# kyle-he/gym-comm

Hardware: AMD Instinct MI355X
Metric: env-steps/sec (whole node) (higher is better)
Workload: dtype int32

## Files before the change

gym-comm_amd/csrc/oc_step_device.h:

```cpp
#pragma once
#include <hip/hip_runtime.h>

#include <type_traits>

#include "../../include/oc_hip.h"
#include "oc_level_host.h"
#include "oc_policy_device.h"

namespace {

#ifdef OC_STAMPS
#define OC_STAMP(k)                                                                  \
  do {                                                                               \
    unsigned long long t_;                                                           \
    __builtin_amdgcn_sched_barrier(0);                                               \
    asm volatile("s_memtime %0\n\ts_waitcnt lgkmcnt(0)" : "=s"(t_)::"memory");     \
    __builtin_amdgcn_sched_barrier(0);                                               \
    oc_tt[(k)] = t_;                                                                 \
  } while (0)
#define OC_STAMP_PARAM , unsigned long long (&oc_tt)[16]
#define OC_STAMP_PASS , oc_tt
#else
#define OC_STAMP(k) do { } while (0)
#define OC_STAMP_PARAM
// ... 136 lines not shown
__device__ __forceinline__ P p_gt(int a, int b) { return p_lt(b, a); }
__device__ __forceinline__ P p_ge(int a, int b) { return ~p_lt(a, b); }
__device__ __forceinline__ P p_le(int a, int b) { return ~p_lt(b, a); }
__device__ __forceinline__ P p_eq_any(int a, int b) { return hide(a == b ? -1 : 0); }
__device__ __forceinline__ P p_gtu_any(unsigned a, unsigned b) { return hide(a > b ? -1 : 0); }
__device__ __forceinline__ P p_geu_any(unsigned a, unsigned b) { return hide(a >= b ? -1 : 0); }
__device__ __forceinline__ P p_ltu_any(unsigned a, unsigned b) { return hide(a < b ? -1 : 0); }
__device__ __forceinline__ P p_bit(int w, unsigned k) { return hide(__builtin_amdgcn_sbfe(w, k, 1u)); }
__device__ __forceinline__ P p_of(bool uniform) { return uniform ? -1 : 0; }
__device__ __forceinline__ int sel(P m, int a, int b) { return (a & m) | (b & ~m); }

__device__ __forceinline__ int iabs(int v) { return v < 0 ? -v : v; }
__device__ __forceinline__ unsigned sad_u32(unsigned a, unsigned b, unsigned c) {
  unsigned r;
  asm("v_sad_u32 %0, %1, %2, %3" : "=v"(r) : "v"(a), "v"(b), "v"(c));
  return r;
}
__device__ __forceinline__ int manhattan(int p, int q) {
  return (int)sad_u32((unsigned)(p & 15), (unsigned)(q & 15), sad_u32((unsigned)(p >> 4), (unsigned)(q >> 4), 0u));
}
__device__ __forceinline__ int px(int p) { return p & 15; }
__device__ __forceinline__ int py(int p) { return p >> 4; }
__device__ __forceinline__ int dense(const Hdr &L, int p) {
  return __mul24(py(p), L.W() - 16) + p;
}
__device__ __forceinline__ int bit128(uint64_t w0, uint64_t w1, int c) {
  const uint64_t v = (c & 64) ? w1 : w0;
  return (int)((v >> (c & 63)) & 1);
}
__device__ __forceinline__ int item_type(const Hdr &L, int i) { return (L.item_types() >> (4 * i)) & 15; }
__device__ __forceinline__ int cell_type(const Hdr &L, int c) {
  if (!L.planes128())
    return (int)((L.cell_lo(0) >> c) & 1) | ((int)((L.cell_hi(0) >> c) & 1) << 1);
  return bit128(L.cell_lo(0), L.cell_lo(1), c) | (bit128(L.cell_hi(0), L.cell_hi(1), c) << 1);
}

#ifdef OC_SPECIALIZED
constexpr bool OC_BORDER_CLOSED = OC_SPEC_HDR.closed_border != 0;
#else
constexpr bool OC_BORDER_CLOSED = false;
#endif

__device__ __forceinline__ double timestep_of(int t, const RunCfg &R) {
  typedef int v2i __attribute__((ext_vector_type(2)));
  const double dt = (double)t;
  const double q0 = dt * R.inv_T;
  const double r = __builtin_fma(-(double)R.T, q0, dt);
  const v2i q = __builtin_bit_cast(v2i, __builtin_fma(r, R.inv_T, q0));
  const P unlimited = p_of(R.T == 0);
  const int hi0 = 0x7FF00000 | (p_z(t) & 0x00080000);
  v2i out;
  out.x = q.x & ~unlimited;
  out.y = sel(unlimited, hi0, q.y);
  return __builtin_bit_cast(double, out);
}


template <int AUX>
struct RowsT {
  __amdgpu_buffer_rsrc_t rsrc;
  int voff;
  int rowbytes;
  __device__ __forceinline__ RowsT(const void *base, int64_t n, int rows, int64_t i, int elem = 4) {
    rsrc = __builtin_amdgcn_make_buffer_rsrc(const_cast<void *>(base), 0, (int)(n * rows * elem), 0x00020000);
    voff = (int)i * elem;
    rowbytes = (int)n * elem;
  }
  __device__ __forceinline__ int ld(int row) const {
    return __builtin_amdgcn_raw_buffer_load_b32(rsrc, voff, row * rowbytes, 0);
  }
  __device__ __forceinline__ void st(int row, int v) const {
    __builtin_amdgcn_raw_buffer_store_b32(v, rsrc, voff, row * rowbytes, AUX);
  }
  __device__ __forceinline__ void st8(int row, int v) const {
    __builtin_amdgcn_raw_buffer_store_b8((char)v, rsrc, voff, row * rowbytes, AUX);
  }
  __device__ __forceinline__ void st_f64(int row, double v) const {
    typedef int v2i __attribute__((ext_vector_type(2)));
    __builtin_amdgcn_raw_buffer_store_b64(__builtin_bit_cast(v2i, v), rsrc, voff, row * rowbytes, AUX);
  }
  __device__ __forceinline__ int soff(int row) const { return row * rowbytes; }
  __device__ __forceinline__ void st_at(int so, int, int v) const {
    __builtin_amdgcn_raw_buffer_store_b32(v, rsrc, voff, so, AUX);
  }
  __device__ __forceinline__ void st8_at(int so, int, int v) const {
    __builtin_amdgcn_raw_buffer_store_b8((char)v, rsrc, voff, so, AUX);
  }
};
template <int AUX, int N>
struct RowsPreT : RowsT<AUX> {
  int so[N > 0 ? N : 1];
  int row0;
  __device__ __forceinline__ RowsPreT(const RowsT<AUX> &rows, int row0_) : RowsT<AUX>(rows), row0(row0_) {
    [[maybe_unused]] int o = row0_ * rows.rowbytes;
#pragma unroll
    for (int k = 0; k < N; k++) {
      so[k] = o;
      asm volatile("" : "+s"(so[k]));
      o = so[k] + rows.rowbytes;
    }
  }
  __device__ __forceinline__ int off(int row) const {
    const int k = row - row0;
    return (k >= 0 && k < N) ? so[k] : row * this->rowbytes;
  }
  __device__ __forceinline__ void st(int row, int v) const {
    __builtin_amdgcn_raw_buffer_store_b32(v, this->rsrc, this->voff, off(row), AUX);
  }
  __device__ __forceinline__ void st8(int row, int v) const {
    __builtin_amdgcn_raw_buffer_store_b8((char)v, this->rsrc, this->voff, off(row), AUX);
  }
  __device__ __forceinline__ void st_v(int row, int vo, int v) const {
    __builtin_amdgcn_raw_buffer_store_b32(v, this->rsrc, vo, off(row), AUX);
  }
  __device__ __forceinline__ void st8_v(int row, int vo, int v) const {
    __builtin_amdgcn_raw_buffer_store_b8((char)v, this->rsrc, vo, off(row), AUX);
  }
};
template <int AUX, int OT>
struct RowsLdsT : RowsT<AUX> {
  float *lds;
  int rowbase, lane;
  __device__ __forceinline__ RowsLdsT(const RowsT<AUX> &rows, float *lds_, int rowbase_, int lane_)
      : RowsT<AUX>(rows), lds(lds_), rowbase(rowbase_), lane(lane_) {}
  __device__ __forceinline__ void st(int row, int v) const {
    RowsT<AUX>::st(row, v);
    lds[(row - rowbase) * 64 + lane] = OT == 2 ? __builtin_bit_cast(float, v) : (float)v;
  }
  __device__ __forceinline__ void st8(int row, int v) const {
    RowsT<AUX>::st8(row, v);
    lds[(row - rowbase) * 64 + lane] = (float)v;
  }
  __device__ __forceinline__ void st_at(int so, int row, int v) const {
    RowsT<AUX>::st_at(so, row, v);
    lds[(row - rowbase) * 64 + lane] = OT == 2 ? __builtin_bit_cast(float, v) : (float)v;
  }
  __device__ __forceinline__ void st8_at(int so, int row, int v) const {
    RowsT<AUX>::st8_at(so, row, v);
    lds[(row - rowbase) * 64 + lane] = (float)v;
  }
};
using Rows = RowsT<0>;
#ifndef OC_AUX_WT
#define OC_AUX_WT 16
#endif
constexpr int AUX_WT = OC_AUX_WT;

template <int B>
struct ShapeIn {
  int ap[B];
  int completed;
  int del_has[MAX_DELS], del_p[MAX_DELS];
  int chop_p[3];
};

template <int M>
__device__ __forceinline__ int pyset_first(const Hdr &L, const uint32_t *__restrict__ probe,
                                           const int (&iw)[M], const bool (&cand)[M], int &has) {
  constexpr int BIG = 1 << 20;
  int ord[M];
#pragma unroll
  for (int i = 0; i < M; i++)
    ord[i] = cand[i] ? (((iw[i] & IW_HOLD) ? 0 : 256) | ((iw[i] >> 16) & 255)) : BIG;
  int cell[3], code[3];
  bool valid[3];
  int prev = -1;
#pragma unroll
  for (int k = 0; k < 3; k++) {
    int cur = BIG, c = 0;
#pragma unroll
    for (int i = 0; i < M; i++) {
      const bool better = ord[i] > prev && ord[i] < cur;
      cur = better ? ord[i] : cur;
      c = better ? ipos(iw[i]) : c;
    }
    valid[k] = cur != BIG;
    cell[k] = c;
    prev = valid[k] ? cur : BIG;
  }
  has = valid[0];
  if (__ballot(valid[1]) == 0) return cell[0];
  valid[1] = valid[1] && cell[1] != cell[0];
  valid[2] = valid[2] && cell[2] != cell[0] && !(valid[1] && cell[2] == cell[1]);
#pragma unroll
  for (int k = 0; k < 3; k++) code[k] = valid[k] ? (int)probe[dense(L, cell[k])] : 0;
  const int s0 = code[0] & 7;
  int s1 = 8, s2 = 8;
#pragma unroll
  for (int t = 7; t >= 0; t--) {
    const int q1 = (code[1] >> (3 * t)) & 7;
    s1 = (q1 != s0) ? q1 : s1;
  }
  s1 = valid[1] ? s1 : 8;
#pragma unroll
  for (int t = 7; t >= 0; t--) {
    const int q2 = (code[2] >> (3 * t)) & 7;
    s2 = (q2 != s0 && q2 != s1) ? q2 : s2;
  }
  s2 = valid[2] ? s2 : 8;
  int best = cell[0], bs = s0;
  best = s1 < bs ? cell[1] : best;
  bs = min(bs, s1);
  best = s2 < bs ? cell[2] : best;
  return best;
}
template <int B>
struct ShapeLoads {
  int d_chop[3][B];
  int d_pair[MAX_PAIRLK];
  int d_del[MAX_DELS][B];
  int d_tile[OC_MAX_DELIV][B];
};

template <int B, int M, bool DUP>
__device__ __forceinline__ void shaping_issue_pos(const Hdr &L, const uint8_t *__restrict__ dist,
                                                  const ShapeIn<B> &in, const int (&ipos)[M], ShapeLoads<B> &ld) {
  const unsigned nc = (unsigned)L.ncells();
  unsigned arow[B];
#pragma unroll
  for (int b = 0; b < B; b++) arow[b] = __umul24((unsigned)dense(L, in.ap[b]), nc);
  unsigned ic[M];
#pragma unroll
  for (int i = 0; i < M; i++) ic[i] = (unsigned)dense(L, ipos[i]);
#pragma unroll
  for (int f = 0; f < 3; f++) {
#pragma unroll
    for (int b = 0; b < B; b++) ld.d_chop[f][b] = 0;
    if (L.chop_mask(f) != 0) {
      unsigned fc = 0;
      if constexpr (DUP) {
        fc = (unsigned)dense(L, in.chop_p[f]);
      } else {
#pragma unroll
        for (int i = 0; i < M; i++) fc = ((int)L.food_item(f) == i) ? ic[i] : fc;
      }
#pragma unroll
      for (int b = 0; b < B; b++) ld.d_chop[f][b] = dist[arow[b] + fc];
    }
  }
#pragma unroll
  for (int k = 0; k < MAX_PAIRLK; k++) {
    ld.d_pair[k] = 0;
    if (k < (int)L.npairlk()) {
      const int li = L.pairlk(k) & 15, lj = (L.pairlk(k) >> 4) & 15;
      unsigned ci = 0, cj = 0;
#pragma unroll
      for (int i = 0; i < M; i++) {
        ci = (li == i) ? ic[i] : ci;
        cj = (lj == i) ? ic[i] : cj;
      }
      ld.d_pair[k] = dist[__umul24(ci, nc) + cj];
    }
  }
#pragma unroll
  for (int k = 0; k < OC_MAX_DELIV; k++) {
#pragma unroll
    for (int b = 0; b < B; b++) ld.d_tile[k][b] = 0;
    if (k < (int)L.ndeliv()) {
      const unsigned dc = (unsigned)dense(L, (int)L.deliv_pos(k));
#pragma unroll
      for (int b = 0; b < B; b++) ld.d_tile[k][b] = dist[arow[b] + dc];
    }
  }
}

template <int B>
__device__ __forceinline__ void shaping_issue_del(const Hdr &L, const uint8_t *__restrict__ dist,
                                                  const ShapeIn<B> &in, ShapeLoads<B> &ld) {
  const unsigned nc = (unsigned)L.ncells();
#pragma unroll
  for (int k = 0; k < MAX_DELS; k++) {
#pragma unroll
    for (int b = 0; b < B; b++) ld.d_del[k][b] = 0;
    if (k < (int)L.ndel()) {
      const unsigned mc = (unsigned)dense(L, in.del_p[k]);
#pragma unroll
      for (int b = 0; b < B; b++) ld.d_del[k][b] = dist[__umul24((unsigned)dense(L, in.ap[b]), nc) + mc];
    }
  }
}

template <int B>
struct ShapeQ {
  double q_chop[B], q_pair, q_del[MAX_DELS][B];
  int nchop, npairs;
  bool del_direct[MAX_DELS][B];
};

__device__ __forceinline__ double quotient(int k, const Hdr &L, double inv_max_path) {
  const double dk = (double)k;
  const double q0 = dk * inv_max_path;
  const double r = __builtin_fma(-(double)L.max_path(), q0, dk);
  return __builtin_fma(r, inv_max_path, q0);
}

template <int B>
__device__ __forceinline__ void shaping_lookup(const Hdr &L, double inv_max_path, const ShapeIn<B> &in,
                                               const ShapeLoads<B> &ld, ShapeQ<B> &q OC_STAMP_PARAM) {
  const int MAXP = L.max_path();
  const int completed = in.completed;
  int d_tile[B];
#pragma unroll
  for (int b = 0; b < B; b++) d_tile[b] = 1 << 20;
#pragma unroll
  for (int k = 0; k < OC_MAX_DELIV; k++)
    if (k < (int)L.ndeliv()) {
#pragma unroll
      for (int b = 0; b < B; b++)
        d_tile[b] = min(d_tile[b], ld.d_tile[k][b] + manhattan(in.ap[b], (int)L.deliv_pos(k)));
    }
  int nchop = 0;
  int mind[B];
#pragma unroll
  for (int b = 0; b < B; b++) mind[b] = 1 << 20;
#pragma unroll
  for (int f = 0; f < 3; f++)
    if (L.chop_mask(f) != 0) {
      const int open = __popc((int)L.chop_mask(f) & ~completed);
      nchop += open;
#pragma unroll
      for (int b = 0; b < B; b++) mind[b] = open ? min(mind[b], ld.d_chop[f][b]) : mind[b];
    }
  int npairs = (int)L.pair_static_max();
  int minpair = npairs ? MAXP : (1 << 20);
  {
    int cur = MAXP;
#pragma unroll
    for (int k = 0; k < MAX_PAIRLK; k++)
      if (k < (int)L.npairlk()) {
        cur = min(cur, ld.d_pair[k]);
        if ((L.pairlk(k) >> 8) & 1) {
          const bool keep = cur != 0;
          npairs += keep ? 1 : 0;
          minpair = keep ? min(minpair, cur) : minpair;
          cur = MAXP;
        }
      }
  }
  int kq_chop[B], kq_pair;
#pragma unroll
  for (int b = 0; b < B; b++) kq_chop[b] = nchop ? (mind[b] + MAXP) + (nchop - 1) * 2 * MAXP : 0;
  kq_pair = nchop ? npairs * MAXP : (npairs ? minpair + (npairs - 1) * MAXP : 0);
  int kq_del[MAX_DELS][B];
#pragma unroll
  for (int k = 0; k < MAX_DELS; k++)
#pragma unroll
    for (int b = 0; b < B; b++) {
      kq_del[k][b] = 0;
      q.del_direct[k][b] = false;
      if (k < (int)L.ndel()) {
        const int d = ld.d_del[k][b] + manhattan(in.ap[b], in.del_p[k]);
        q.del_direct[k][b] = d == 0;
        kq_del[k][b] = d == 0 ? d_tile[b] : d;
      }
    }
#pragma unroll
  for (int b = 0; b < B; b++) q.q_chop[b] = quotient(kq_chop[b], L, inv_max_path);
  q.q_pair = quotient(kq_pair, L, inv_max_path);
#pragma unroll
  for (int k = 0; k < MAX_DELS; k++)
#pragma unroll
    for (int b = 0; b < B; b++) q.q_del[k][b] = (k < (int)L.ndel()) ? quotient(kq_del[k][b], L, inv_max_path) : 0.0;
  q.nchop = nchop;
  q.npairs = npairs;
  OC_STAMP(4);
}

template <int B>
__device__ __forceinline__ void shaping_sum(const Hdr &L, const ShapeIn<B> &in, const ShapeQ<B> &q,
                                            double &s0, double &s1 OC_STAMP_PARAM) {
  double tot[B];
#pragma unroll
  for (int b = 0; b < B; b++) {
    tot[b] = q.nchop ? q.q_chop[b] : 0.0;
    tot[b] = q.npairs ? tot[b] + q.q_pair : tot[b];
  }
#pragma unroll
  for (int k = 0; k < MAX_DELS; k++)
    if (k < (int)L.ndel()) {
      const bool open = !((in.completed >> L.del_bit(k)) & 1);
#pragma unroll
      for (int b = 0; b < B; b++) {
        const double add = !in.del_has[k] ? 2.0 : (q.del_direct[k][b] ? q.q_del[k][b] : q.q_del[k][b] + 1.0);
        tot[b] = open ? tot[b] + add : tot[b];
      }
    }
  s0 = tot[0];
  s1 = B > 1 ? tot[1] : 0.0;
  OC_STAMP(6);
}

template <int A, int M, bool DUP, int PM, bool FLAT>
__device__ __forceinline__ void env_step(const Hdr &L, const RunCfg &R, const uint8_t *__restrict__ dist,
                                         const uint32_t *__restrict__ probe,
                                         Env<A, M, DUP> &e, const int (&act_in)[A], int &reward, int &done, P &done_p,
                                         int &success, ShapeIn<(A < 2 ? A : 2)> &sin,
                                         ShapeLoads<(A < 2 ? A : 2)> &sld OC_STAMP_PARAM) {
  const int W = L.W(), H = L.H();
  const auto pb = [](int w, unsigned k) -> P {
    if constexpr (PM == 2 && FLAT) return __builtin_amdgcn_sbfe(w, k, 1u);
    return p_bit(w, k);
  };
  e.t = min(e.t + 1, 0xFFFF);
  static_assert(OC_ACT_NOOP == 4 && OC_FLOOR == 0 && OC_COUNTER == 1 && OC_CUTBOARD == 2 && OC_DELIVERY == 3, "codes");

  int act[A], np[A], tgt_p[A];
  P moving[A], t_nonfloor[A], t_deliv[A], t_cutb[A];
#pragma unroll
  for (int a = 0; a < A; a++) {
    int c = act_in[a];
    e.err |= p_gtu_any((unsigned)c, 4u) & OC_ERR_ACTION;
    c = (int)min((unsigned)c, 4u);
    act[a] = c;
    moving[a] = p_ne(c, OC_ACT_NOOP);
    int cell;
    P oob = 0;
    if constexpr (OC_BORDER_CLOSED) {
      constexpr uint64_t STEP = 0x0001FFF010ull;
      const int q = e.ap[a] + (int)(int8_t)(STEP >> (8 * c));
      tgt_p[a] = q;
      cell = dense(L, q);
    } else {
      const int dx = (c == OC_ACT_RIGHT) - (c == OC_ACT_LEFT);
      const int dy = (c == OC_ACT_DOWN) - (c == OC_ACT_UP);
      const int qx = px(e.ap[a]) + dx, qy = py(e.ap[a]) + dy;
      oob = ~(p_ltu_any((unsigned)qx, (unsigned)W) & p_ltu_any((unsigned)qy, (unsigned)H));
      e.err |= oob & OC_ERR_OOB;
      const int tx = min(max(qx, 0), W - 1), ty = min(max(qy, 0), H - 1);
      tgt_p[a] = tx | (ty << 4);
      cell = ty * W + tx;
    }
    P lo, hi;
    if (!L.planes128()) {
      lo = pb((int)(L.cell_lo(0) >> cell), 0);
      hi = pb((int)(L.cell_hi(0) >> cell), 0);
    } else {
      lo = -bit128(L.cell_lo(0), L.cell_lo(1), cell);
      hi = -bit128(L.cell_hi(0), L.cell_hi(1), cell);
    }
    t_nonfloor[a] = lo | hi;
    t_deliv[a] = lo & hi;
    t_cutb[a] = hi & ~lo;
    np[a] = sel(t_nonfloor[a] | oob, e.ap[a], tgt_p[a]);
  }
  P ex[A];
#pragma unroll
  for (int a = 0; a < A; a++) ex[a] = -1;
#pragma unroll
  for (int i = 0; i < A; i++)
#pragma unroll
    for (int j = i + 1; j < A; j++) {
      const P same = p_eq(np[i], np[j]);
      const P i_stays = p_eq(np[i], e.ap[i]) & moving[i];
      const P j_stays = p_eq(np[j], e.ap[j]) & moving[j];
      const P swap = p_eq(e.ap[i], np[j]) & p_eq(e.ap[j], np[i]);
      const P block_i = sel(same, ~i_stays, swap);
      const P block_j = sel(same, i_stays | ~j_stays, swap);
      ex[i] &= ~block_i;
      ex[j] &= ~block_j;
    }

  const P play = p_of(PM == 2 ? R.play != 0 : PM == 1);
#pragma unroll
  for (int a = 0; a < A; a++) {
    const P acting = ex[a] & moving[a];
    const int pa = e.ap[a];
    const int tp = tgt_p[a];
    const int held_g = A == 2 ? hide(e.ahp[a] - 1) : e.ahp[a] - 1;
    const P holding = A == 2 ? ~hide(held_g >> 31) : p_nz(e.ahp[a]);
    const int hold_code = (a + 1) << 12;
    int held_or = 0, tgt_or = 0;
    P mine[M], tgt[M];
#pragma unroll
    for (int i = 0; i < M; i++) {
      const int w = e.iw[i];
      const int u = item_type(L, i) != OC_PLATE ? (w ^ IW_CHOP) : w;
      mine[i] = A == 2 ? pb(w, 12 + a) : p_eq(w & IW_HOLD, hold_code);
      tgt[i] = p_eq(w & (IW_HOLD | IW_POS), tp);
      held_or |= mine[i] & u;
      tgt_or |= tgt[i] & u;
    }
    const P tgt_any = p_nz(tgt_or);
    P held_multi;
    if constexpr (DUP) {
      int nm = 0;
#pragma unroll
      for (int i = 0; i < M; i++) nm -= mine[i];
      held_multi = p_gt(nm, 1);
    } else {
      held_multi = p_nz(held_or & IW_TSET & ((held_or & IW_TSET) - (1 << 24)));
    }
    const P held_fresh = pb(held_or, 8);
    const P any_fresh = pb(held_or | tgt_or, 8);
    const P two_plates = p_nz((held_or & tgt_or) & sig_of_type<DUP>(OC_PLATE));
    const P at_deliv = t_deliv[a];
    const P nf = acting & t_nonfloor[a];
    const P do_move = acting & ~t_nonfloor[a];
    const P nfh = nf & holding & ~at_deliv, nfe = nf & ~holding & ~at_deliv;
    const P do_deliver = nf & holding & at_deliv & held_multi & ~held_fresh;
    const P mergeable = ~(two_plates | any_fresh);
    const P do_merge = nfh & tgt_any & mergeable;
    const P chop_here = t_cutb[a] & ~held_multi & held_fresh & ~play;
    const P do_chop = nfh & ~tgt_any & chop_here;
    const P do_drop = nfh & ~tgt_any & ~chop_here;
    const P chop_there = nfe & tgt_any & play & t_cutb[a] & pb(tgt_or, 8);
    const P do_pick = nfe & tgt_any & ~chop_there & p_of(!((R.allergic >> a) & 1));
    const P put = do_deliver | do_drop | (do_merge & play);
    const P take = (do_merge & ~play) | do_pick;
    const int newg = (int)min((unsigned)held_g, (unsigned)igrp(tgt_or));
    int objf;
    if constexpr (DUP) {
      const int newsig = (held_or & TS<true>) + (tgt_or & TS<true>);
      const int seq4 = M + e.mctr;
      int kf = 0;
#pragma unroll
      for (int j = 0; j < MAX_NAMES; j++)
        if (j < (int)L.nnames()) {
          const P hit = p_eq(newsig >> 24, (int)L.name_sig(j));
          const int sh = 4 * (j & 7);
          const int cur = (e.kn[j >> 3] >> sh) & 15;
          kf = sel(hit, cur, kf);
          const P enter = hit & p_z(cur);
          e.kn[j >> 3] |= enter & do_merge & ((seq4 + 1) << sh);
        }
      const int kseq = sel(p_nz(kf), kf - 1, seq4);
      objf = newsig | (newg << 9) | (((kseq << 4) | seq4) << 16);
    } else {
      objf = ((held_or | tgt_or) & IW_TSET) | (newg << 9) | ((M + e.mctr) << 16);
    }
    if (A > 2) {
      P shared = 0;
#pragma unroll
      for (int b = 0; b < A; b++)
        if (b != a) shared |= p_eq(e.ap[b], pa);
      if (__ballot((shared & do_merge) != 0) != 0) {
        P alias = 0;
#pragma unroll
        for (int j = 0; j < M; j++) {
          const int w = e.iw[j];
          alias |= p_nz(w & IW_HOLD) & p_ne(w & IW_HOLD, hold_code) & p_eq(ipos(w), pa) &
                   p_z((w ^ held_or) & TS<DUP>) & p_gt(w & IW_SEQ, held_or & IW_SEQ);
        }
        e.err |= shared & do_merge & alias & OC_ERR_ALIAS;
      }
    }
    const int mask_m = ((do_move | put) & IW_POS) | (put & IW_HOLD) | (do_merge & OBJ<DUP>) | (do_chop & IW_CHOP);
    const int mask_t = (take & (IW_POS | IW_HOLD)) | (do_merge & OBJ<DUP>) | (chop_there & IW_CHOP);
    const int val_m = tp | IW_CHOP | objf;
    const int val_t = pa | hold_code | objf | IW_CHOP;
#pragma unroll
    for (int i = 0; i < M; i++) {
      const int selm = (mine[i] & mask_m) | (tgt[i] & mask_t);
      e.iw[i] = bfi(selm, sel(mine[i], val_m, val_t), e.iw[i]);
    }
    e.ap[a] = sel(do_move, tp, pa);
    e.ahp[a] = sel(take, newg + 1, e.ahp[a]) & ~put;
    e.mctr -= do_merge;
  }

  constexpr int B = A < 2 ? A : 2;
#pragma unroll
  for (int b = 0; b < B; b++) sin.ap[b] = e.ap[b];
  if constexpr (DUP) {
#pragma unroll
    for (int f = 0; f < 3; f++) {
      sin.chop_p[f] = 0;
      if (L.chop_mask(f) != 0) {
        bool cand[M];
#pragma unroll
        for (int i = 0; i < M; i++) cand[i] = ((L.food_items(f) >> i) & 1) && !(e.iw[i] & IW_CHOP);
        int has;
        sin.chop_p[f] = pyset_first<M>(L, probe, e.iw, cand, has);
      }
    }
  }
  {
    int ipb[M];
#pragma unroll
    for (int i = 0; i < M; i++) ipb[i] = ipos(e.iw[i]);
    shaping_issue_pos<B, M, DUP>(L, dist, sin, ipb, sld);
    __builtin_amdgcn_sched_barrier(0);
  }
  OC_STAMP(2);
  const int d0 = (int)L.deliv_pos(0);
  int present = 0, at_delivery = 0;
  P rep_ok[M];
#pragma unroll
  for (int i = 0; i < M; i++) {
    const int w = e.iw[i];
    const P rep = p_eq(w & IW_GRP, i << 9);
    const P lone_fresh = item_type(L, i) != OC_PLATE
                             ? p_eq(w & (TS<DUP> | IW_CHOP), sig_of_type<DUP>(item_type(L, i))) : 0;
    rep_ok[i] = rep & ~lone_fresh;
    if constexpr (!DUP) {
      const int b = rep_ok[i] & (1 << itset(w));
      present |= b;
      at_delivery |= p_eq(ipos(w), d0) & b;
    }
  }
  int cnt_mask = 0, del_mask = 0, newly;
  if constexpr (DUP) {
    int rose = 0;
#pragma unroll
    for (int g = 0; g < MAX_GOALS; g++)
      if (g < (int)L.ngoal()) {
        int cnt = 0;
        P hasd = 0;
        P m[M];
#pragma unroll
        for (int i = 0; i < M; i++) {
          m[i] = rep_ok[i] & p_eq(e.iw[i] & TS<true>, (int)L.goal_sig(g) << 24);
          P seen = 0;
#pragma unroll
          for (int j = 0; j < i; j++) seen |= m[j] & p_eq(ipos(e.iw[j]), ipos(e.iw[i]));
          cnt -= m[i] & ~seen;
          hasd |= m[i] & p_eq(ipos(e.iw[i]), d0);
        }
        cnt = min(cnt, 3);
        const int old = (e.goalcnt >> (2 * g)) & 3;
        rose |= p_gt(cnt, old) & (int)L.goal_nd(g);
        cnt_mask |= cnt << (2 * g);
        del_mask |= hasd & (int)L.goal_dl(g);
      }
    newly = rose;
  } else {
#pragma unroll
    for (int g = 0; g < MAX_GOALS; g++) {
      if (g < (int)L.ngoal()) {
        cnt_mask |= pb(present, L.goal_tset(g)) & (int)L.goal_nd(g);
        del_mask |= pb(at_delivery, L.goal_tset(g)) & (int)L.goal_dl(g);
      }
    }
    newly = cnt_mask & ~e.goalcnt;
  }
  reward = __popc(newly) + 3 * __popc(del_mask);
  e.completed |= newly | del_mask;
  e.goalcnt = cnt_mask;
  P timeout;
  if constexpr (FLAT) timeout = p_ge(e.t, R.T != 0 ? (int)R.T : 0x10000);
  else timeout = R.T != 0 ? p_ge(e.t, R.T) : 0;
  const P all_delivered = p_eq_any(del_mask, (int)L.deliver_mask());
  done_p = hide(timeout | all_delivered);
  done = done_p & 1;
  success = (~timeout & all_delivered) & 1;

  sin.completed = e.completed;
#pragma unroll
  for (int k = 0; k < MAX_DELS; k++) {
    sin.del_has[k] = 0;
    sin.del_p[k] = 0;
    if (k < (int)L.ndel()) {
      if constexpr (DUP) {
        bool cand[M];
#pragma unroll
        for (int i = 0; i < M; i++)
          cand[i] = (rep_ok[i] & p_eq(e.iw[i] & TS<true>, (int)L.del_sig(k) << 24)) != 0;
        sin.del_p[k] = pyset_first<M>(L, probe, e.iw, cand, sin.del_has[k]);
      } else {
#pragma unroll
        for (int i = 0; i < M; i++) {
          const P ok = rep_ok[i] & p_eq(e.iw[i] & IW_TSET, (int)L.del_tset(k) << 24);
          sin.del_has[k] |= ok & 1;
          sin.del_p[k] = sel(ok, ipos(e.iw[i]), sin.del_p[k]);
        }
      }
    }
  }
  shaping_issue_del<B>(L, dist, sin, sld);
  __builtin_amdgcn_sched_barrier(0);
  OC_STAMP(3);
}

#ifdef OC_SPECIALIZED
constexpr int OBS_NSLOT = OC_SPEC_HDR.S > 0 ? OC_SPEC_HDR.S : 1;
#else
constexpr int OBS_NSLOT = 1;
#endif
struct ObsSlots {
  int sh[OBS_NSLOT];
  __device__ __forceinline__ ObsSlots(const RunCfg &R, bool pin) {
#ifdef OC_SPECIALIZED
#pragma unroll
    for (int s = 0; s < (int)OC_SPEC_HDR.S; s++) {
      sh[s] = R.slot_identity ? s : (int)((R.slot4[s >> 2] >> (8 * (s & 3))) & 31);
      if (pin) asm volatile("" : "+s"(sh[s]));
    }
#else
    sh[0] = 0;
#endif
  }
};

template <int A, int M, bool DUP, int OT, typename OutRows>
__device__ __forceinline__ void env_obs(const Hdr &L, const RunCfg &R, const ObsSlots &slots, const Env<A, M, DUP> &e,
                                        int viewer, int radius, bool viewer_blind, bool ego_blind, int C, int comm0,
                                        int comm1, const OutRows &out, int row0) {
  const int vp = viewer == 0 ? e.ap[0] : e.ap[1];
  const int vhp = viewer == 0 ? e.ahp[0] : e.ahp[1];
  const int vx = px(vp), vy = py(vp);
  int ddx[4], ddy[4], st[4], hid[4];
  int loc[4];
  if (viewer_blind) {
#pragma unroll
    for (int ch = 0; ch < 4; ch++) ddx[ch] = ddy[ch] = st[ch] = loc[ch] = 0, hid[ch] = 1;
  } else {
#pragma unroll
    for (int ch = 0; ch < 4; ch++) {
      int bw = 0;
      bool any = false;
#pragma unroll
      for (int i = 0; i < M; i++)
        if (item_type(L, i) == ch) {
          bw = (!any || (e.iw[i] & IW_SEQ) > (bw & IW_SEQ)) ? e.iw[i] : bw;
          any = true;
        }
// ... 508 lines not shown
      __builtin_amdgcn_make_buffer_rsrc(p.out, 0, (int)(2 * 7 * Q * p.n * 4), 0x00020000);
  int aq[A], abyte[A];
#pragma unroll
  for (int a = 0; a < A; a++) {
    const int c = (int)__umul24((unsigned)px(e.ap[a]), (unsigned)H) + py(e.ap[a]);
    aq[a] = c >> 2;
    abyte[a] = 8 * (c & 3);
  }
  int iq[M], ishift[M], ival[M];
#pragma unroll
  for (int m = 0; m < M; m++) {
    const int pos = ipos(e.iw[m]);
    const int c = (int)__umul24((unsigned)px(pos), (unsigned)H) + py(pos);
    iq[m] = c >> 2;
    ishift[m] = 8 * (c & 3);
    ival[m] = item_type(L, m) == OC_PLATE ? 1 : ichop(e.iw[m]) + 1;
    bool later = false;
#pragma unroll
    for (int o = 0; o < M; o++)
      if (o != m && item_type(L, o) == item_type(L, m))
        later |= ipos(e.iw[o]) == pos && (e.iw[o] & IW_SEQ) > (e.iw[m] & IW_SEQ);
    iq[m] = later ? -1 : iq[m];
  }
  const int vx[2] = {px(e.ap[0]), px(e.ap[1])}, vy[2] = {py(e.ap[0]), py(e.ap[1])};
  int x = 0, y = 0;
  for (int q = 0; q < Q; q++) {
    unsigned fog[2] = {0u, 0u}, tile = 0u;
#pragma unroll
    for (int b = 0; b < 4; b++)
      if (4 * q + b < ncell) {
        tile |= (unsigned)cell_type(L, y * W + x) << (8 * b);
#pragma unroll
        for (int v = 0; v < 2; v++)
          fog[v] |= (int)sad_u32((unsigned)x, (unsigned)vx[v], sad_u32((unsigned)y, (unsigned)vy[v], 0u)) > p.radius
                        ? 0xFFu << (8 * b) : 0u;
        if (++y == H) y = 0, x++;
      }
#pragma unroll
    for (int k = 0; k < 7; k++) {
      unsigned val = k == 0 ? tile : 0u;
      if (k >= 3) {
#pragma unroll
        for (int m = 0; m < M; m++)
          if (item_type(L, m) + 3 == k)
            val |= iq[m] == q ? (unsigned)ival[m] << ishift[m] : 0u;
      }
      if (k >= 1 && k <= A) {
        const int a = k - 1;
        val = aq[a] == q ? (val & ~(0xFFu << abyte[a])) | (1u << abyte[a]) : val;
      }
#pragma unroll
      for (int v = 0; v < 2; v++)
        __builtin_amdgcn_raw_buffer_store_b32((int)(val | fog[v]), rsrc, (int)i * 4,
                                              (int)(((v * 7 + k) * Q + q) * p.n * 4), AUX_WT);
    }
  }
  p.holding[i] = e.ahp[0] != 0;
  p.holding[p.n + i] = e.ahp[1] != 0;
}

struct ResetArgs {
  LevelHdr L;
  const void *tables;
  int32_t n16, quot_bytes;
  int32_t *state;
  const int32_t *mask;
  const int32_t *placement;
  uint32_t *rng;
  int64_t n;
};

template <int A, int M, bool DUP>
__global__ void __launch_bounds__(256) k_reset(const ResetArgs p) {
  OC_HDR_LOAD(p);
  const int64_t i = (int64_t)blockIdx.x * blockDim.x + threadIdx.x;
  if (i >= p.n) return;
  if (p.mask != nullptr && p.mask[i] == 0) return;
  constexpr int WS = state_words<A, M, DUP>();
  const Tables tb = stage_tables<false>(p.tables, p.n16, p.quot_bytes);
  int32_t w[WS];
#pragma unroll
  for (int r = 0; r < WS; r++) w[r] = L.init_words(r);
  place_items<A, M, WS>(L, tb, p.placement, p.rng, p.n, i, w);
#pragma unroll
  for (int r = 0; r < WS; r++) p.state[(int64_t)r * p.n + i] = w[r];
}

__global__ void __launch_bounds__(256) k_random_actions(uint32_t *rng, int32_t *move_row, int32_t *comm_row,
                                                        uint32_t num_comm, int64_t n) {
  const int64_t i = (int64_t)blockIdx.x * blockDim.x + threadIdx.x;
  if (i >= n) return;
  uint32_t st = rng[i];
  move_row[i] = (int32_t)__umulhi(pcg32(st), 4u);
  comm_row[i] = (int32_t)__umulhi(pcg32(st), num_comm);
  rng[i] = st;
}

struct MultiArgs {
  LevelHdr L;
  RunCfg R;
  const void *tables;
  int32_t n16, quot_bytes;
  int32_t *state;
  int32_t *comm;
  const int32_t *actions;
  void *obs;
  double *timestep;
  double *reward;
  int32_t *done;
  int32_t *sparse;
  int64_t *metrics;
  const int32_t *placement;
  uint32_t *rng;
  oc_step_opts opt;
  int64_t n;
  int32_t auto_reset;
  oc_wrap_cfg cfg;
  oc_step_policy pol[2];
  int32_t pol_ksteps;
  unsigned long long *timeline;
  int64_t timeline_stride;
};

constexpr int DUTY_STATE = 1, DUTY_SHAPE = 2, DUTY_OBS0 = 4, DUTY_OBS1 = 8, DUTY_ALL = 15;

template <int ROWS>
__device__ __forceinline__ float *pol_lds_feat() {
  __shared__ float a[2 * ROWS * 64];
  return a;
}
__device__ __forceinline__ float *pol_lds_ts() {
  __shared__ float t[64];
  return t;
}

template <int M, bool LDS, int OT, bool WT, bool DUP, int XO, int DUTY, bool SPLIT, bool POL = false, int LN = 1>
__device__ __forceinline__ void multi_step_body(int32_t *const state_, const int32_t *const actions_,
                                                int32_t *const comm_, int64_t *const metrics_,
                                                const int32_t n_, const int32_t block_, const void *const ego_src_,
                                                const void *const alt_src_, const MultiArgs &p) {
  constexpr int A = 2;
  constexpr bool D_STATE = (DUTY & DUTY_STATE) != 0, D_SHAPE = (DUTY & DUTY_SHAPE) != 0;
  using Out = RowsT<WT ? AUX_WT : 0>;
#ifdef OC_SPECIALIZED
  constexpr int POL_ROWS = (POL && SPLIT) ? 22 + OC_SPEC_HDR.S + 8 : 1;
#else
  constexpr int POL_ROWS = 1;
#endif
  OC_HDR_LOAD(p);
  static_assert(LN == 1 || (SPLIT && XO == 0 && !POL && !LDS && DUTY != DUTY_ALL), "lane-split: the plain four-way split only");
  constexpr int EPW = 64 / LN;
  const int i = SPLIT ? (int)blockIdx.x * EPW + (int)(threadIdx.x & (EPW - 1))
                      : (int)blockIdx.x * (block_ & 0xFFFF) + (int)threadIdx.x;
  constexpr bool PART0_ONLY = LN > 1 && (DUTY & (DUTY_OBS0 | DUTY_OBS1)) == 0;
  const bool valid = PART0_ONLY ? (i < (int)n_ && (int)(threadIdx.x & 63) < EPW) : i < (int)n_;
  const bool ego_from_pairs = XO != 0 && ((block_ >> 16) & 1), alt_from_pairs = XO != 0 && ((block_ >> 17) & 1),
             alt_from_rng = XO != 0 && ((block_ >> 18) & 1), pairs64 = XO != 0 && ((block_ >> 19) & 1);
#ifdef OC_STAMPS
  unsigned long long oc_tt[16];
  for (int k = 0; k < 16; k++) oc_tt[k] = 0;
#endif
  OC_STAMP(0);
  Tables tb;
  if constexpr (LDS) tb = stage_tables<true>(p.tables, p.n16, p.quot_bytes);
  MetricsSlot slot(metrics_, i);
  int reward = 0, done = 0, success = 0, comp = 0;
  bool err = false;
  constexpr int POL_MINE = (DUTY == DUTY_OBS0) ? 0 : (DUTY == DUTY_OBS1) ? 2 : (DUTY == DUTY_STATE) ? 1 : 3;
  constexpr int POL_VIEWER = POL_MINE >> 1;
  [[maybe_unused]] ocpol::Weights pol_w;
  if constexpr (POL && SPLIT) {
    ocpol::load_weights(pol_w, p.pol[POL_VIEWER].w1, p.pol[POL_VIEWER].w2, p.pol[POL_VIEWER].b2,
                        (int)threadIdx.x & 63, p.pol_ksteps);
  }
  if (valid) {
    constexpr int WS = state_words<A, M, DUP>();
    const Out st(state_, n_, WS, i), cm(comm_, n_, 2, i);
    int32_t w[WS];
#pragma unroll
    for (int r = 0; r < WS; r++) w[r] = st.ld(r);
    typedef int v2i __attribute__((ext_vector_type(2)));
    typedef int v4i __attribute__((ext_vector_type(4)));
    v4i eq = {0, 0, 0, 0}, aq = {0, 0, 0, 0};
    v2i er = {0, 0}, ar = {0, 0};
    uint32_t alt_rs = 0;
    if constexpr (XO != 0) {
      const auto desc = [&](const void *base, bool on, int bytes) {
        return __builtin_amdgcn_make_buffer_rsrc(const_cast<void *>(base), 0, on ? bytes : 0, 0x00020000);
      };
      const int sh = pairs64 ? 4 : 3;
      const __amdgpu_buffer_rsrc_t d_er = desc(actions_, !ego_from_pairs, (int)n_ * 16),
                                   d_ar = desc(actions_, !alt_from_pairs && !alt_from_rng, (int)n_ * 16),
                                   d_eq = desc(ego_src_, ego_from_pairs, (int)n_ << sh),
                                   d_aq = desc(alt_src_, alt_from_pairs && !alt_from_rng, (int)n_ << sh),
                                   d_rs = desc(alt_src_, alt_from_rng, (int)n_ * 4);
      const int off4 = i << 2, offq = i << sh, row = (int)n_ * 4;
      eq = (v4i)__builtin_amdgcn_raw_buffer_load_b128(d_eq, offq, 0, 0);
      aq = (v4i)__builtin_amdgcn_raw_buffer_load_b128(d_aq, offq, 0, 0);
      alt_rs = (uint32_t)__builtin_amdgcn_raw_buffer_load_b32(d_rs, off4, 0, 0);
      er.x = __builtin_amdgcn_raw_buffer_load_b32(d_er, off4, 0, 0);
      er.y = __builtin_amdgcn_raw_buffer_load_b32(d_er, off4, row, 0);
      ar.x = __builtin_amdgcn_raw_buffer_load_b32(d_ar, off4, 2 * row, 0);
      ar.y = __builtin_amdgcn_raw_buffer_load_b32(d_ar, off4, 3 * row, 0);
    } else {
      const Rows ac(actions_, n_, 4, i);
      er.x = ac.ld(0), er.y = ac.ld(1);
      ar.x = ac.ld(2), ar.y = ac.ld(3);
    }
    if constexpr (!LDS) tb = stage_tables<false>(p.tables, p.n16, p.quot_bytes);
    asm volatile("" ::"s"(tb.dist), "s"(p.obs), "s"(p.timestep), "s"(p.reward), "s"(p.done),
                 "s"(p.sparse), "s"(p.auto_reset), "s"(p.R.inv_T), "s"(p.R.inv_max_path));
    if constexpr (XO != 0) asm volatile("" ::"s"(p.opt.ep_return), "s"(p.opt.ep_length));
#if defined(OC_SPECIALIZED) && !defined(OC_SPEC_GEOMETRY)
    asm volatile("" ::"s"(L.W()), "s"(L.ncells()), "s"(L.max_path()), "s"(L.cell_lo(0)), "s"(L.cell_hi(0)),
                 "s"(L.deliv_pos(0)));
#endif
    double ep_ret = 0.0;
    int ep_len = 0, prev_done = 0;
    if (XO != 0 && p.opt.ep_return != nullptr) {
      const Rows er(p.opt.ep_return, n_, 1, i, 8);
      ep_ret = __builtin_bit_cast(double, (v2i)__builtin_amdgcn_raw_buffer_load_b64(er.rsrc, er.voff, 0, 0));
      ep_len = Rows(p.opt.ep_length, n_, 1, i).ld(0);
      prev_done = Rows(p.done, n_, 1, i).ld(0);
    }
    Env<A, M, DUP> e;
    unpack<A, M, DUP>(e, w);
    const int C = p.cfg.obs.num_comm;
    const int F = 22 + L.S() + 2 * C;
    const Out ob(p.obs, p.n, 2 * F, i, OT == 1 ? 1 : 4);
    constexpr bool OBS_ONLY = SPLIT && (DUTY == DUTY_OBS0 || DUTY == DUTY_OBS1);
#ifdef OC_TS_OBS1
    constexpr int TS_DUTY = POL ? DUTY_OBS0 : DUTY_OBS1;
#else
    constexpr int TS_DUTY = DUTY_OBS0;
#endif
#ifdef OC_SPECIALIZED
    constexpr int NPRE_ALL = 22 + (int)OC_SPEC_HDR.S + 8;
    constexpr int NPRE = (OBS_ONLY && !POL && XO == 0) ? (NPRE_ALL < 40 ? NPRE_ALL : 40) : 0;
#else
    constexpr int NPRE = 0;
#endif
    const ObsSlots slots(p.R, NPRE != 0);
    const RowsPreT<WT ? AUX_WT : 0, NPRE> obp(ob, DUTY == DUTY_OBS1 ? F : 0);
    if constexpr (NPRE != 0) asm volatile("" ::"s"(ob.rsrc));
#ifdef OC_SPECIALIZED
    using Parts = std::conditional_t<(LN > 1 && OBS_ONLY), LaneParts<(LN > 1 ? LN : 2)>, NoParts>;
    [[maybe_unused]] const Parts parts(ob, slots, C);
#endif
    const Out tso(p.timestep, p.n, 1, i, 8);
    if constexpr (NPRE != 0 && DUTY == TS_DUTY) asm volatile("" ::"s"(tso.rsrc), "v"(tso.voff));
    uint32_t place_rs = 0;
    if constexpr (SPLIT) {
      if (L.nscatter() != 0 && p.rng != nullptr) place_rs = (uint32_t)Rows(p.rng, n_, 1, i).ld(0);
      if constexpr (XO != 0)
        asm volatile("s_waitcnt vmcnt(0)\n\ts_barrier" : "+v"(eq), "+v"(aq), "+v"(er), "+v"(ar), "+v"(alt_rs)::"memory");
      else asm volatile("s_waitcnt vmcnt(0)\n\ts_barrier" ::: "memory");
      __builtin_amdgcn_s_waitcnt(WAIT_VMCNT0);
      if constexpr (NPRE != 0) __builtin_amdgcn_sched_barrier(0);
    } else if constexpr (XO != 0) {
      asm volatile("" : "+v"(eq), "+v"(aq), "+v"(er), "+v"(ar), "+v"(alt_rs));
    }
    int ego_mv = er.x, ego_cm = er.y, alt_mv = ar.x, alt_cm = ar.y;
    if constexpr (XO != 0) {
      const auto narrow = [](int lo, int hi) { return lo | ~p_eq_any(hi, lo >> 31); };
      if (pairs64) {
        ego_mv |= narrow(eq.x, eq.y), ego_cm |= narrow(eq.z, eq.w);
        alt_mv |= narrow(aq.x, aq.y), alt_cm |= narrow(aq.z, aq.w);
      } else {
        ego_mv |= eq.x, ego_cm |= eq.y;
        alt_mv |= aq.x, alt_cm |= aq.y;
      }
    }
    if (alt_from_rng) {
      alt_mv = (int)__umulhi(pcg32(alt_rs), 4u);
      alt_cm = (int)__umulhi(pcg32(alt_rs), (uint32_t)p.cfg.obs.num_comm);
      if (!SPLIT || D_STATE) {
        Rows(alt_src_, n_, 1, i).st(0, (int)alt_rs);
        if (p.opt.alt_played != nullptr) {
          const Rows ap(p.opt.alt_played, n_, 2, i);
          ap.st(0, alt_mv);
          ap.st(1, alt_cm);
        }
      }
    }
    OC_STAMP(1);
    const bool cfg_comm_on = XO == 2 ? p.cfg.communication_on != 0 : true, cfg_ego_led = XO == 2 ? p.cfg.ego_led != 0 : false;
    const int cfg_can_move = XO == 2 ? p.cfg.can_move_mask : 3, cfg_ego_idx = XO == 2 ? p.cfg.ego_agent_idx : 0;
    const int cfg_blind = XO == 2 ? p.cfg.obs.blind_mask : 0;
    const unsigned NC = (unsigned)p.cfg.obs.num_comm;
    const bool ego_talks = cfg_comm_on, alt_talks = cfg_comm_on && !cfg_ego_led;
    const P ego_cm_bad = p_geu_any((unsigned)ego_cm, NC), alt_cm_bad = p_geu_any((unsigned)alt_cm, NC);
    const P bad_cm = (p_of(ego_talks) & ego_cm_bad) | (p_of(alt_talks) & alt_cm_bad);
    const int c0 = ego_talks ? (ego_cm | ego_cm_bad) : -1;
    const int c1 = alt_talks ? (alt_cm | alt_cm_bad) : -1;
    if constexpr (D_STATE) {
      cm.st(0, c0);
      cm.st(1, c1);
    }
    const P bad_mv = p_gtu_any((unsigned)ego_mv, 3u) | p_gtu_any((unsigned)alt_mv, 3u);
    const int em = (cfg_can_move & 1) ? (int)min((unsigned)ego_mv, 4u) : OC_ACT_NOOP;
    const int am = (cfg_can_move & 2) ? (int)min((unsigned)alt_mv, 4u) : OC_ACT_NOOP;
    int act[A];
    act[0] = cfg_ego_idx == 0 ? em : am;
    act[1] = cfg_ego_idx == 0 ? am : em;
    const int err_before = e.err;
    P done_p = 0;
    e.err |= (bad_mv | bad_cm) & OC_ERR_ACTION;
    ShapeIn<2> sin;
    ShapeLoads<2> sld;
    env_step<A, M, DUP, XO == 2 ? 2 : 0, SPLIT>(L, p.R, tb.dist, tb.probe, e, act, reward, done, done_p, success, sin, sld OC_STAMP_PASS);
    comp = e.completed;
    err = e.err != err_before;
    if constexpr (D_STATE) {
      Out(p.done, p.n, 1, i).st(0, done);
#ifndef OC_STAMPS
      if (p.sparse != nullptr) Out(p.sparse, p.n, 1, i).st(0, reward);
#endif
    }
    if constexpr (DUTY != DUTY_SHAPE) {
      if ((DUTY & (DUTY_OBS0 | DUTY_OBS1)) == 0 && L.nscatter() == 0) {
        pack<A, M, DUP>(e, w);
        const P fresh = done_p & p_of(p.auto_reset != 0);
#pragma unroll
        for (int r = 0; r < WS; r++) w[r] = sel(fresh, L.init_words(r), w[r]);
      } else if (OBS_ONLY && L.nscatter() == 0) {
        int32_t w0[WS];
#pragma unroll
        for (int r = 0; r < WS; r++) w0[r] = L.init_words(r);
        Env<A, M, DUP> e0;
        unpack<A, M, DUP>(e0, w0);
        const P fresh = done_p & p_of(p.auto_reset != 0);
#pragma unroll
        for (int a = 0; a < A; a++) e.ap[a] = sel(fresh, e0.ap[a], e.ap[a]), e.ahp[a] = sel(fresh, e0.ahp[a], e.ahp[a]);
#pragma unroll
        for (int k = 0; k < M; k++) e.iw[k] = sel(fresh, e0.iw[k], e.iw[k]);
        e.t = sel(fresh, e0.t, e.t);
        e.completed = sel(fresh, e0.completed, e.completed);
      } else if (done && p.auto_reset) {
#pragma unroll
        for (int r = 0; r < WS; r++) w[r] = L.init_words(r);
        if constexpr (SPLIT) {
          place_items_from<A, M, WS>(L, tb, p.placement, p.rng != nullptr, place_rs, p.n, i, w);
          if (D_STATE && L.nscatter() != 0 && p.rng != nullptr) p.rng[i] = place_rs;
        } else {
          place_items<A, M, WS>(L, tb, p.placement, p.rng, p.n, i, w);
        }
        unpack<A, M, DUP>(e, w);
      } else {
        pack<A, M, DUP>(e, w);
      }
    }
    if constexpr (D_STATE) {
#pragma unroll
      for (int r = 0; r < WS; r++) st.st(r, w[r]);
    }
    constexpr bool TS_MINE = OBS_ONLY ? DUTY == TS_DUTY : (DUTY & DUTY_OBS0) != 0;
    [[maybe_unused]] double tsd = 0.0;
    if constexpr (TS_MINE && OBS_ONLY && !POL) tsd = timestep_of(e.t, p.R);
    if constexpr (TS_MINE && OBS_ONLY && !POL) tso.st_f64(0, tsd);
    ShapeQ<2> sq;
    if constexpr (D_SHAPE) shaping_lookup<2>(L, p.R.inv_max_path, sin, sld, sq OC_STAMP_PASS);
    const bool ego_blind = cfg_blind & 1;
    if constexpr (POL && SPLIT) {
      const int ln = (int)threadIdx.x & 63;
      if constexpr ((DUTY & DUTY_OBS0) != 0) {
        const RowsLdsT<WT ? AUX_WT : 0, OT> obl(ob, pol_lds_feat<POL_ROWS>(), 0, ln);
        env_obs<A, M, DUP, OT>(L, p.R, slots, e, 0, p.cfg.obs.fow_radius, cfg_blind & 1, ego_blind, C, c0, c1, obl, 0);
        const double tsd = timestep_of(e.t, p.R);
        Out(p.timestep, p.n, 1, i, 8).st_f64(0, tsd);
        pol_lds_ts()[ln] = (float)tsd;
      }
      if constexpr ((DUTY & DUTY_OBS1) != 0) {
        const RowsLdsT<WT ? AUX_WT : 0, OT> obl(ob, pol_lds_feat<POL_ROWS>() + POL_ROWS * 64, F, ln);
        env_obs<A, M, DUP, OT>(L, p.R, slots, e, 1, p.cfg.obs.fow_radius, (cfg_blind >> 1) & 1, ego_blind, C, c0, c1, obl, F);
      }
    } else {
#ifdef OC_SPECIALIZED
      if constexpr (LN > 1) {
        if constexpr (DUTY == DUTY_OBS0) env_obs_lanes<A, M, DUP, OT, LN>(L, parts, e, 0, p.cfg.obs.fow_radius, C, c0, c1, obp, 0);
        if constexpr (DUTY == DUTY_OBS1) env_obs_lanes<A, M, DUP, OT, LN>(L, parts, e, 1, p.cfg.obs.fow_radius, C, c0, c1, obp, F);
      } else
#endif
      {
        if constexpr ((DUTY & DUTY_OBS0) != 0)
          env_obs<A, M, DUP, OT>(L, p.R, slots, e, 0, p.cfg.obs.fow_radius, cfg_blind & 1, ego_blind, C, c0, c1, obp, 0);
        if constexpr ((DUTY & DUTY_OBS1) != 0)
          env_obs<A, M, DUP, OT>(L, p.R, slots, e, 1, p.cfg.obs.fow_radius, (cfg_blind >> 1) & 1, ego_blind, C, c0, c1, obp, F);
      }
      if constexpr (TS_MINE && !OBS_ONLY) tso.st_f64(0, timestep_of(e.t, p.R));
    }
    OC_STAMP(5);
    if constexpr (D_SHAPE) {
      double s0, s1;
      shaping_sum<2>(L, sin, sq, s0, s1 OC_STAMP_PASS);
      const double shaped = ((double)reward - s0) - s1;
      Out(p.reward, p.n, 1, i, 8).st_f64(0, shaped);
      if (XO != 0 && p.opt.ep_return != nullptr) {
        Out(p.opt.ep_return, p.n, 1, i, 8).st_f64(0, prev_done ? shaped : ep_ret + shaped);
        Out(p.opt.ep_length, p.n, 1, i).st(0, prev_done ? 1 : ep_len + 1);
      }
    }
  }
  OC_STAMP(7);
  if constexpr (D_STATE) slot.add(metrics_ != nullptr, valid, done, success, reward, comp, err);
  OC_STAMP(8);
  if constexpr (POL) {
    static_assert(XO != 0, "the fused policies belong to the variants with action sources");
    if constexpr (SPLIT) asm volatile("s_waitcnt lgkmcnt(0)\n\ts_barrier" ::: "memory");
    else asm volatile("s_waitcnt vmcnt(0)" ::: "memory");
    const int lane = (int)threadIdx.x & 63;
    const int C = p.cfg.obs.num_comm, F = 22 + L.S() + 2 * C;
    const uint32_t n32 = (uint32_t)n_;
    constexpr int ELEM = OT == 1 ? 1 : 4;
#pragma unroll
    for (int v = 0; v < 2; v++)
#pragma unroll
      for (int q = 0; q < 2; q++) {
        if (SPLIT && (2 * v + q) != POL_MINE) continue;
        const int64_t env0 = (int64_t)(i & ~63) + 32 * q + (lane & 31);
        const bool ok = env0 < n_;
        const uint32_t env = (uint32_t)(ok ? env0 : n_ - 1);
        const void *rows = (const char *)p.obs + (size_t)v * F * n_ * ELEM;
        int32_t *pairs = (int32_t *)const_cast<void *>(v == 0 ? ego_src_ : alt_src_);
        if constexpr (SPLIT) {
          const int col = 32 * q + (lane & 31);
          ocpol::policy_pass<OT, 4, true, true>(rows, n32, env, ok, lane, p.pol[v].w1, p.pol[v].w2, p.pol[v].b2,
                                                p.pol[v].rng, pairs, nullptr, pol_lds_ts()[col], F, C, p.pol_ksteps,
                                                pol_lds_feat<POL_ROWS>() + v * POL_ROWS * 64, col, &pol_w);
        } else {
          ocpol::policy_pass<OT, 4>(rows, n32, env, ok, lane, p.pol[v].w1, p.pol[v].w2, p.pol[v].b2, p.pol[v].rng,
                                    pairs, nullptr, (float)p.timestep[env], F, C, p.pol_ksteps);
        }
      }
  }
#ifdef OC_STAMPS
  if ((threadIdx.x & 63) == 0 && p.sparse != nullptr) {
    long long *dbg = (long long *)p.sparse + ((int64_t)blockIdx.x * (blockDim.x >> 6) + (threadIdx.x >> 6)) * 16;
    for (int k = 0; k < 16; k++) dbg[k] = (long long)oc_tt[k];
  }
#endif
}

template <int M, bool LDS, int OT, bool WT, bool DUP, int XO, int SP, bool POL = false, int LN = 1>
__global__ void __launch_bounds__(256) k_multi_step(int32_t *const state_, const int32_t *const actions_,
                                                    int32_t *const comm_, int64_t *const metrics_,
                                                    const int32_t n_, const int32_t block_,
                                                    const void *const ego_src_, const void *const alt_src_,
                                                    const MultiArgs p) {
  static_assert(SP == 1 || SP == 2 || SP == 4, "waves per 64 envs");
  static_assert(SP != 2 || !POL, "the fused policies need the four-wave split");
  static_assert(SP == 1 || !LDS, "the split launch reads the tables from global memory");
  static_assert(LN == 1 || (SP == 4 && XO == 0 && !POL), "lanes per env: the plain four-way split only");
  OC_TL_BEGIN();
#ifdef OC_SPECIALIZED
  const MultiArgs &pk = p;
#else
  struct KernArgs { int32_t *a; const int32_t *b; int32_t *c; int64_t *d; int32_t n, blk; const void *e, *f; MultiArgs p; };
  [[maybe_unused]] const MultiArgs &pk = *reinterpret_cast<const MultiArgs *>(
      reinterpret_cast<const char *>((const void *)__builtin_amdgcn_kernarg_segment_ptr()) + offsetof(KernArgs, p));
#endif
#define OC_BODY(duty) multi_step_body<M, LDS, OT, WT, DUP, XO, (duty), true, POL, LN>(state_, actions_, comm_, metrics_, n_, block_, ego_src_, alt_src_, pk)
  if constexpr (SP == 1) {
    multi_step_body<M, LDS, OT, WT, DUP, XO, DUTY_ALL, false, POL>(state_, actions_, comm_, metrics_, n_, block_, ego_src_, alt_src_, p);
  } else {
    const int role = __builtin_amdgcn_readfirstlane((int)threadIdx.x >> 6);
    if constexpr (SP == 2) {
      if (role == 0) OC_BODY(DUTY_STATE | DUTY_OBS0);
      else OC_BODY(DUTY_SHAPE | DUTY_OBS1);
    } else {
      if (role == 0) OC_BODY(DUTY_OBS0);
      else if (role == 1) OC_BODY(DUTY_OBS1);
      else if (role == 2) OC_BODY(DUTY_STATE);
      else OC_BODY(DUTY_SHAPE);
    }
  }
#undef OC_BODY
  OC_TL_END(p.timeline, p.timeline_stride, LN);
}

}
```

Baseline: 1.620 billion.

## Split shaping work across lane halves, one agent per lane

```diff
diff --git a/gym-comm_amd/csrc/oc_step_device.h b/gym-comm_amd/csrc/oc_step_device.h
--- a/gym-comm_amd/csrc/oc_step_device.h
+++ b/gym-comm_amd/csrc/oc_step_device.h
@@ -312,6 +312,7 @@
   int completed;
   int del_has[MAX_DELS], del_p[MAX_DELS];
   int chop_p[3];
+  P part;
 };
 
 template <int M>
@@ -550,12 +551,12 @@
   OC_STAMP(6);
 }
 
-template <int A, int M, bool DUP, int PM, bool FLAT>
+template <int A, int M, bool DUP, int PM, bool FLAT, int SB = (A < 2 ? A : 2)>
 __device__ __forceinline__ void env_step(const Hdr &L, const RunCfg &R, const uint8_t *__restrict__ dist,
                                          const uint32_t *__restrict__ probe,
                                          Env<A, M, DUP> &e, const int (&act_in)[A], int &reward, int &done, P &done_p,
-                                         int &success, ShapeIn<(A < 2 ? A : 2)> &sin,
-                                         ShapeLoads<(A < 2 ? A : 2)> &sld OC_STAMP_PARAM) {
+                                         int &success, ShapeIn<SB> &sin,
+                                         ShapeLoads<SB> &sld OC_STAMP_PARAM) {
   const int W = L.W(), H = L.H();
   const auto pb = [](int w, unsigned k) -> P {
     if constexpr (PM == 2 && FLAT) return __builtin_amdgcn_sbfe(w, k, 1u);
@@ -718,9 +719,14 @@
     e.mctr -= do_merge;
   }
 
-  constexpr int B = A < 2 ? A : 2;
-#pragma unroll
-  for (int b = 0; b < B; b++) sin.ap[b] = e.ap[b];
+  constexpr int B = SB;
+  static_assert(SB == (A < 2 ? A : 2) || (SB == 1 && A >= 2), "sim agents per lane");
+  if constexpr (SB == 1 && A >= 2) {
+    sin.ap[0] = sel(sin.part, e.ap[1], e.ap[0]);
+  } else {
+#pragma unroll
+    for (int b = 0; b < B; b++) sin.ap[b] = e.ap[b];
+  }
   if constexpr (DUP) {
 #pragma unroll
     for (int f = 0; f < 3; f++) {
@@ -1535,8 +1541,13 @@
   constexpr int EPW = 64 / LN;
   const int i = SPLIT ? (int)blockIdx.x * EPW + (int)(threadIdx.x & (EPW - 1))
                       : (int)blockIdx.x * (block_ & 0xFFFF) + (int)threadIdx.x;
-  constexpr bool PART0_ONLY = LN > 1 && (DUTY & (DUTY_OBS0 | DUTY_OBS1)) == 0;
-  const bool valid = PART0_ONLY ? (i < (int)n_ && (int)(threadIdx.x & 63) < EPW) : i < (int)n_;
+#ifndef OC_LS_SHAPE
+#define OC_LS_SHAPE 1
+#endif
+  constexpr bool LS_SHAPE = LN > 1 && DUTY == DUTY_SHAPE && OC_LS_SHAPE != 0;
+  constexpr bool PART0_ONLY = LN > 1 && (DUTY & (DUTY_OBS0 | DUTY_OBS1)) == 0 && !LS_SHAPE;
+  [[maybe_unused]] const bool part0 = (int)(threadIdx.x & 63) < EPW;
+  const bool valid = PART0_ONLY ? (i < (int)n_ && part0) : i < (int)n_;
   const bool ego_from_pairs = XO != 0 && ((block_ >> 16) & 1), alt_from_pairs = XO != 0 && ((block_ >> 17) & 1),
              alt_from_rng = XO != 0 && ((block_ >> 18) & 1), pairs64 = XO != 0 && ((block_ >> 19) & 1);
 #ifdef OC_STAMPS
@@ -1632,6 +1643,11 @@
 #endif
     const Out tso(p.timestep, p.n, 1, i, 8);
     if constexpr (NPRE != 0 && DUTY == TS_DUTY) asm volatile("" ::"s"(tso.rsrc), "v"(tso.voff));
+    [[maybe_unused]] P part_hi = 0;
+    if constexpr (LS_SHAPE) {
+      part_hi = p_bit((int)threadIdx.x, 5);
+      asm volatile("" : "+v"(part_hi));
+    }
     uint32_t place_rs = 0;
     if constexpr (SPLIT) {
       if (L.nscatter() != 0 && p.rng != nullptr) place_rs = (uint32_t)Rows(p.rng, n_, 1, i).ld(0);
@@ -1639,7 +1655,7 @@
         asm volatile("s_waitcnt vmcnt(0)\n\ts_barrier" : "+v"(eq), "+v"(aq), "+v"(er), "+v"(ar), "+v"(alt_rs)::"memory");
       else asm volatile("s_waitcnt vmcnt(0)\n\ts_barrier" ::: "memory");
       __builtin_amdgcn_s_waitcnt(WAIT_VMCNT0);
-      if constexpr (NPRE != 0) __builtin_amdgcn_sched_barrier(0);
+      if constexpr (NPRE != 0 || LS_SHAPE) __builtin_amdgcn_sched_barrier(0);
     } else if constexpr (XO != 0) {
       asm volatile("" : "+v"(eq), "+v"(aq), "+v"(er), "+v"(ar), "+v"(alt_rs));
     }
@@ -1689,8 +1705,10 @@
     const int err_before = e.err;
     P done_p = 0;
     e.err |= (bad_mv | bad_cm) & OC_ERR_ACTION;
-    ShapeIn<2> sin;
-    ShapeLoads<2> sld;
+    constexpr int SB = LS_SHAPE ? 1 : 2;
+    ShapeIn<SB> sin;
+    ShapeLoads<SB> sld;
+    sin.part = part_hi;
     env_step<A, M, DUP, XO == 2 ? 2 : 0, SPLIT>(L, p.R, tb.dist, tb.probe, e, act, reward, done, done_p, success, sin, sld OC_STAMP_PASS);
     comp = e.completed;
     err = e.err != err_before;
@@ -1741,8 +1759,8 @@
     [[maybe_unused]] double tsd = 0.0;
     if constexpr (TS_MINE && OBS_ONLY && !POL) tsd = timestep_of(e.t, p.R);
     if constexpr (TS_MINE && OBS_ONLY && !POL) tso.st_f64(0, tsd);
-    ShapeQ<2> sq;
-    if constexpr (D_SHAPE) shaping_lookup<2>(L, p.R.inv_max_path, sin, sld, sq OC_STAMP_PASS);
+    ShapeQ<SB> sq;
+    if constexpr (D_SHAPE) shaping_lookup<SB>(L, p.R.inv_max_path, sin, sld, sq OC_STAMP_PASS);
     const bool ego_blind = cfg_blind & 1;
     if constexpr (POL && SPLIT) {
       const int ln = (int)threadIdx.x & 63;
@@ -1775,9 +1793,16 @@
     OC_STAMP(5);
     if constexpr (D_SHAPE) {
       double s0, s1;
-      shaping_sum<2>(L, sin, sq, s0, s1 OC_STAMP_PASS);
+      shaping_sum<SB>(L, sin, sq, s0, s1 OC_STAMP_PASS);
+      if constexpr (LS_SHAPE) {
+        const v2i mine = __builtin_bit_cast(v2i, s0);
+        v2i other;
+        other.x = (int)__builtin_amdgcn_permlane32_swap((unsigned)mine.x, (unsigned)mine.x, false, false)[1];
+        other.y = (int)__builtin_amdgcn_permlane32_swap((unsigned)mine.y, (unsigned)mine.y, false, false)[1];
+        s1 = __builtin_bit_cast(double, other);
+      }
       const double shaped = ((double)reward - s0) - s1;
-      Out(p.reward, p.n, 1, i, 8).st_f64(0, shaped);
+      if (!LS_SHAPE || part0) Out(p.reward, p.n, 1, i, 8).st_f64(0, shaped);
       if (XO != 0 && p.opt.ep_return != nullptr) {
         Out(p.opt.ep_return, p.n, 1, i, 8).st_f64(0, prev_done ? shaped : ep_ret + shaped);
         Out(p.opt.ep_length, p.n, 1, i).st(0, prev_done ? 1 : ep_len + 1);
```

Measured after the change: 1.572 billion. 0.97x the previous value.
